# michelbarbeau/gr-uwspr

Hardware: NVIDIA B200
Metric: WSPR windows/sec (coarse+fine sync+demod) (higher is better)
Workload: dtype f32

## Files before the change

### gr-uwspr_b200/csrc/capi.cu

```cuda
#include <limits.h>
#include <math.h>
#include <stdio.h>
#include <stdlib.h>
#include <string.h>

#include <algorithm>
#include <chrono>
#include <future>
#include <string>
#include <thread>
#include <vector>

#include "common.cuh"
#include "../host/wspr_tables.h"

#ifndef M_PI
#define M_PI 3.14159265358979323846
#endif

namespace {

const int kMaxChunks = 1024;
const int kCounterSets = 15;
const int kCounterInts = 4 + 4 * kCounterSets;

struct UwChunk {
    int w0, nw, set, slot, cset, group, strm;
    size_t xoff;
};

struct Knobs {
    int host_chunk = 0;
    int tail_groups = 2;
    int tail_piece = 0;
    bool no_tail_split = false;
    bool no_early_d2h = false;
    bool trace = false;
    bool no_fine_reuse = false;
    int dev_chunks = 1;
    int fine_ctas_per_sm = 0;
    int fine_slice = 16384;
    int fine_slice_side = 16384;
};

Knobs read_knobs()
{
    Knobs k;
    auto geti = [](const char *name, int def) {
        const char *e = getenv(name);
        return e ? atoi(e) : def;
    };
    k.host_chunk = std::max(0, geti("UWSPR_B200_HOST_CHUNK", k.host_chunk));
    k.tail_groups = std::max(0, std::min(2, geti("UWSPR_B200_TAIL_GROUPS", k.tail_groups)));
    k.tail_piece = std::max(0, geti("UWSPR_B200_TAIL_PIECE", 0));
    k.no_tail_split = getenv("UWSPR_B200_NO_TAIL_SPLIT") != nullptr;
    k.no_early_d2h = getenv("UWSPR_B200_NO_EARLY_D2H") != nullptr;
    k.trace = getenv("UWSPR_B200_TRACE") != nullptr;
    k.no_fine_reuse = getenv("UWSPR_B200_NO_FINE_REUSE") != nullptr;
    k.dev_chunks = std::max(1, geti("UWSPR_B200_DEV_CHUNKS", 1));
    k.fine_ctas_per_sm = std::max(0, geti("UWSPR_B200_FINE_CTAS_PER_SM", 0));
    k.fine_slice = std::max(1, geti("UWSPR_B200_FINE_SLICE", k.fine_slice));
    k.fine_slice_side = std::max(1, geti("UWSPR_B200_FINE_SLICE_SIDE", k.fine_slice_side));
    return k;
}

struct Buffers {
    float2 *x_stage[3] = { nullptr, nullptr, nullptr };
    size_t x_stage_elems = 0;
    float *amp = nullptr;
    float *ps_dbg = nullptr;
    float *psavg = nullptr;
    UwPeak *peaks = nullptr;
    int *npk = nullptr;
    int *base = nullptr;
    size_t win_cap = 0;
    UwItem *items = nullptr;
    uwspr_b200_candidate_t *cands = nullptr;
    uwspr_b200_refined_t *refined = nullptr;
    uwspr_b200_jiggle_t *jig = nullptr;
    uint8_t *soft = nullptr;
    int *fine_tickets = nullptr;
    void *fine_state[3] = { nullptr, nullptr, nullptr };
    void *fine_pbuf[3] = { nullptr, nullptr, nullptr };
    void *fine_pe[3] = { nullptr, nullptr, nullptr };
    void *fine_pbest[3] = { nullptr, nullptr, nullptr };
    void *fine_tables[3] = { nullptr, nullptr, nullptr };
    int *counters = nullptr;
    float *window = nullptr;
    float2 *twiddle = nullptr;
    uint32_t *off4 = nullptr;
    short *hyp_unique = nullptr;
    int *dec_first_ok = nullptr;
    int *dec_tasks = nullptr;
    uint32_t *dec_task_cycles = nullptr;
    unsigned long long *dec_task_msg = nullptr;
    int *dec_counters = nullptr;
    uint8_t *dec_out = nullptr;
    short *mettab = nullptr;
    uint8_t *rows = nullptr;
    size_t rows_cap = 0;
};

}

struct uwspr_b200_ctx {
    uwspr_b200_params_t prm;
    UwDims d;
    Buffers b;
    int device = 0, sm_count = 0;
    int chunk_windows = 0, max_windows = 0, max_candidates = 0;
    int grid_coarse = 0, grid_points = 0, grid_lags = 0;
    int fine_slice[3] = { 0, 0, 0 };
    cudaStream_t compute = nullptr, compute2 = nullptr, compute3 = nullptr, copy = nullptr, d2h = nullptr;
    int *h_ends = nullptr;
    bool own_compute = true;
    cudaEvent_t ev_h2d[3] = { nullptr, nullptr, nullptr }, ev_free[3] = { nullptr, nullptr, nullptr }, ev_wl[3] = { nullptr, nullptr, nullptr };
    cudaEvent_t ev_fork = nullptr, ev_join = nullptr, ev_join3 = nullptr;
    int last_cw = 0;
    std::vector<UwChunk> last_chunks;
    Knobs knobs;
    int last_sets = 1;
    std::vector<cudaEvent_t> ev;
    cudaEvent_t ev_begin = nullptr, ev_end = nullptr;
    cudaEvent_t ev_cp0 = nullptr, ev_cp1 = nullptr, ev_kend = nullptr;
    float ms[4] = { 0, 0, 0, 0 };
    int64_t launches = 0;
    std::string err;
    bool debug_ps = false;
    bool have_coarse = false;
    bool have_fine = false;
    int last_jig_count = 0;
    int fano_grid = 0;
    int last_nwin = 0, last_total = 0;
    const float *last_samples = nullptr;
    int64_t last_stride = 0;
    std::future<int> pending;
};

namespace {

int fail(uwspr_b200_ctx *c, int status, const std::string &msg)
{
    if (c) c->err = msg;
    return status;
// ... 274 lines not shown
        const float2 *xfine = xdev + uw_window_offset(geom, 0);
        const size_t so = (size_t)s * cw + (size_t)ch.slot;
        float *amp = b.amp + so * d.n_rows * d.nbp;
        float *psd = (ctx->debug_ps && b.ps_dbg) ? b.ps_dbg + so * d.n_rows * d.nbp : nullptr;
        float *psavg = b.psavg + so * d.nbp;
        UwPeak *peaks = b.peaks + so * d.maxcand;
        int *set = b.counters + 4 + 4 * ch.cset;
        cudaEvent_t *e = &ctx->ev[4 * c];
        CU(cudaEventRecord(e[0], st));
        if (do_coarse) {
            uw_launch_spectrogram(d, xdev, geom, nw, b.window, b.twiddle, amp, psd, psavg, peaks,
                                  b.npk + w0, st);
            ctx->launches++;
        }
        CU(cudaEventRecord(e[1], st));
        if (c >= 1 && chunks[c - 1].strm != ch.strm) CU(cudaStreamWaitEvent(st, ctx->ev_wl[chunks[c - 1].strm], 0));
        uw_launch_worklist(b.npk + w0, nw, ctx->max_candidates, b.base + w0, b.items, b.counters, set, st);
        ctx->launches++;
        if (streams[1] != cs) CU(cudaEventRecord(ctx->ev_wl[ch.strm], st));
        if (early) CU(cudaMemcpyAsync(&ctx->h_ends[c], set + 2, sizeof(int), cudaMemcpyDeviceToHost, st));
        if (do_coarse) {
            uw_launch_coarse(d, amp, peaks, b.items, set + 2, ctx->max_candidates, b.off4, b.hyp_unique, b.cands, set,
                             ctx->grid_coarse, st);
            ctx->launches++;
        }
        CU(cudaEventRecord(e[2], st));
        if (do_fine) {
            const long long most = std::min<long long>(ctx->max_candidates, (long long)nw * d.maxcand);
            const int slice = ctx->fine_slice[ch.strm];
            for (long long s0 = 0; s0 < most; s0 += slice)
                ctx->launches += uw_launch_fine(d, xfine, geom, b.items, set + 1, set + 2, ctx->max_candidates, b.cands,
                                                jig_first, jig_count, b.refined, b.jig, b.soft, (int)s0, slice,
                                                b.fine_state[ch.strm], b.fine_pbuf[ch.strm], b.fine_pe[ch.strm], b.fine_pbest[ch.strm], b.fine_tables[ch.strm], b.fine_tickets + 16 * ch.strm, ctx->grid_points,
                                                ctx->grid_lags, kn.no_fine_reuse ? 0 : 1, st);
        }
        CU(cudaEventRecord(e[3], st));
        if (host) CU(cudaEventRecord(ctx->ev_free[s], st));
    }
    if (streams[1] != cs) {
        CU(cudaEventRecord(ctx->ev_join, streams[1]));
        CU(cudaStreamWaitEvent(cs, ctx->ev_join, 0));
        if (use3) {
            CU(cudaEventRecord(ctx->ev_join3, streams[2]));
            CU(cudaStreamWaitEvent(cs, ctx->ev_join3, 0));
        }
    }
    ctx->last_cw = cw;
    ctx->last_sets = nsets;
    if (ctx->knobs.trace) CU(cudaEventRecord(ctx->ev_kend, cs));
    int done = 0;
    auto fetch = [&](int lo, int hi, cudaStream_t q) -> cudaError_t {
        cudaError_t e = cudaSuccess;
        const size_t n = (size_t)(hi - lo);
        if (hi <= lo) return e;
        if (cands_out && do_coarse && e == cudaSuccess)
            e = cudaMemcpyAsync(cands_out + lo, b.cands + lo, sizeof(uwspr_b200_candidate_t) * n, cudaMemcpyDeviceToHost, q);
        if (do_fine && refined_out && e == cudaSuccess)
            e = cudaMemcpyAsync(refined_out + lo, b.refined + lo, sizeof(uwspr_b200_refined_t) * n, cudaMemcpyDeviceToHost, q);
        if (do_fine && jig_out && e == cudaSuccess)
            e = cudaMemcpyAsync(jig_out + (size_t)lo * jig_count, b.jig + (size_t)lo * jig_count,
                                sizeof(uwspr_b200_jiggle_t) * n * jig_count, cudaMemcpyDeviceToHost, q);
        if (do_fine && soft_out && e == cudaSuccess)
            e = cudaMemcpyAsync(soft_out + (size_t)lo * jig_count * UW_NSYM, b.soft + (size_t)lo * jig_count * UW_NSYM,
                                n * jig_count * UW_NSYM, cudaMemcpyDeviceToHost, q);
        return e;
    };
    if (early) {
// ... 182 lines not shown
    }
    CUC(cudaMalloc(&b.window, UW_FFT_N * sizeof(float)));
    CUC(cudaMalloc(&b.twiddle, UW_FFT_N * sizeof(float2)));
    CUC(cudaMalloc(&b.off4, off4.size() * sizeof(uint32_t)));
    CUC(cudaMalloc(&b.hyp_unique, hyp_unique.size() * sizeof(short)));
    CUC(cudaMemcpy(b.window, window.data(), UW_FFT_N * sizeof(float), cudaMemcpyHostToDevice));
    CUC(cudaMemcpy(b.twiddle, tw.data(), UW_FFT_N * sizeof(float2), cudaMemcpyHostToDevice));
    CUC(cudaMemcpy(b.off4, off4.data(), off4.size() * sizeof(uint32_t), cudaMemcpyHostToDevice));
    CUC(cudaMemcpy(b.hyp_unique, hyp_unique.data(), hyp_unique.size() * sizeof(short), cudaMemcpyHostToDevice));
    CUC(cudaStreamCreateWithFlags(&ctx->compute, cudaStreamNonBlocking));
    CUC(cudaStreamCreateWithFlags(&ctx->copy, cudaStreamNonBlocking));
    CUC(cudaStreamCreateWithFlags(&ctx->compute2, cudaStreamNonBlocking));
    CUC(cudaStreamCreateWithFlags(&ctx->d2h, cudaStreamNonBlocking));
    CUC(cudaStreamCreateWithFlags(&ctx->compute3, cudaStreamNonBlocking));
    CUC(cudaEventCreateWithFlags(&ctx->ev_join3, cudaEventDisableTiming));
    CUC(cudaHostAlloc(&ctx->h_ends, sizeof(int) * (kMaxChunks + 4), cudaHostAllocDefault));
    CUC(cudaEventCreateWithFlags(&ctx->ev_fork, cudaEventDisableTiming));
    CUC(cudaEventCreateWithFlags(&ctx->ev_join, cudaEventDisableTiming));
    for (int q = 0; q < 3; q++) {
        CUC(cudaEventCreateWithFlags(&ctx->ev_h2d[q], cudaEventDisableTiming));
        CUC(cudaEventCreateWithFlags(&ctx->ev_free[q], cudaEventDisableTiming));
        CUC(cudaEventCreateWithFlags(&ctx->ev_wl[q], cudaEventDisableTiming));
    }
    CUC(cudaEventCreate(&ctx->ev_begin));
    CUC(cudaEventCreate(&ctx->ev_cp0));
    CUC(cudaEventCreate(&ctx->ev_cp1));
    CUC(cudaEventCreate(&ctx->ev_kend));
    CUC(cudaEventCreate(&ctx->ev_end));
    if (uw_coarse_setup(d) || uw_fine_setup() || uw_fano_setup())
        return bail(fail(ctx, UWSPR_B200_E_CUDA, "cannot reserve shared memory for the kernels (not an sm_100a device?)"));
    ctx->grid_coarse = ctx->sm_count * uw_coarse_blocks_per_sm(d);
    ctx->fano_grid = ctx->sm_count * uw_fano_blocks_per_sm();
    {
        int bp = 1, bl = 1;
        uw_fine_blocks_per_sm(&bp, &bl);
        if (ctx->knobs.fine_ctas_per_sm > 0) {
            bp = std::min(bp, ctx->knobs.fine_ctas_per_sm);
            bl = std::min(bl, ctx->knobs.fine_ctas_per_sm);
        }
        ctx->grid_points = ctx->sm_count * bp;
        ctx->grid_lags = ctx->sm_count * bl;
        if (ctx->knobs.trace)
            fprintf(stderr, "uwspr_b200 trace: fine path: %d + %d resident CTAs per SM (points, lags), slices of %d candidates\n", bp, bl,
                    std::max(1, std::min(ctx->max_candidates, ctx->knobs.fine_slice)));
    }
    CUC(cudaDeviceSynchronize());
#undef CUC
    *ctx_out = ctx;
    return UWSPR_B200_OK;
}

void uwspr_b200_destroy(uwspr_b200_ctx *ctx)
{
    if (!ctx) return;
    if (ctx->pending.valid()) ctx->pending.wait();
    cudaSetDevice(ctx->device);
    Buffers &b = ctx->b;
    void *ptrs[] = { b.x_stage[0], b.x_stage[1], b.x_stage[2], b.amp, b.ps_dbg, b.psavg, b.peaks, b.npk, b.base, b.items,
                     b.cands, b.refined, b.jig, b.soft, b.counters, b.fine_tickets, b.fine_state[0], b.fine_state[1], b.fine_state[2], b.fine_pbuf[0], b.fine_pbuf[1],
                     b.fine_pbuf[2], b.fine_pe[0], b.fine_pe[1], b.fine_pe[2], b.fine_pbest[0], b.fine_pbest[1], b.fine_pbest[2], b.fine_tables[0], b.fine_tables[1], b.fine_tables[2], b.window, b.twiddle, b.off4, b.hyp_unique,
                     b.dec_first_ok, b.dec_tasks, b.dec_task_cycles, b.dec_task_msg, b.dec_counters, b.dec_out, b.mettab, b.rows };
    for (void *q : ptrs)
        if (q) cudaFree(q);
    for (cudaEvent_t e : ctx->ev) cudaEventDestroy(e);
    for (int q = 0; q < 3; q++) {
        if (ctx->ev_h2d[q]) cudaEventDestroy(ctx->ev_h2d[q]);
        if (ctx->ev_free[q]) cudaEventDestroy(ctx->ev_free[q]);
        if (ctx->ev_wl[q]) cudaEventDestroy(ctx->ev_wl[q]);
    }
    if (ctx->ev_begin) cudaEventDestroy(ctx->ev_begin);
    if (ctx->ev_cp0) cudaEventDestroy(ctx->ev_cp0);
    if (ctx->ev_cp1) cudaEventDestroy(ctx->ev_cp1);
    if (ctx->ev_kend) cudaEventDestroy(ctx->ev_kend);
    if (ctx->ev_end) cudaEventDestroy(ctx->ev_end);
    if (ctx->compute && ctx->own_compute) cudaStreamDestroy(ctx->compute);
    if (ctx->copy) cudaStreamDestroy(ctx->copy);
    if (ctx->compute2) cudaStreamDestroy(ctx->compute2);
// ... 347 lines not shown
```

### gr-uwspr_b200/csrc/common.cuh

```cuda
#pragma once

#include <cuda_runtime.h>
#include <stdint.h>

#include "uwspr_b200.h"

#define UW_NSYM 162
#define UW_FFT_N 512
#define UW_HOP 128
#define UW_NK0 26
#define UW_NIFR 5
#define UW_NTRAJ 125
#define UW_SPS 256
#define UW_NP 45000
#define UW_MAX_TILE_W 40
#define UW_MAX_UNIQUE 192
#define UW_NQUAD 41

struct UwDims {
    int fl, n_rows, size, m, hpbm, finpb, noiseidx, maxfreqs, maxcand, maxdrift, cf;
    float df, min_snr, floor_val, threshold;
    int bin_lo, n_bins, nbp;
    int n_lin, n_hyp, n_unique;
    int off_min, off_max, tile_w;
// ... 55 lines not shown
}
__device__ __forceinline__ uw_f2 uw_sub2(uw_f2 a, uw_f2 b)
{
    uw_f2 r;
    asm("sub.rn.f32x2 %0, %1, %2;" : "=l"(r) : "l"(a), "l"(b));
    return r;
}
__device__ __forceinline__ uw_f2 uw_mul2(uw_f2 a, uw_f2 b, uw_f2 nz)
{
    uw_f2 r;
    asm("fma.rn.f32x2 %0, %1, %2, %3;" : "=l"(r) : "l"(a), "l"(b), "l"(nz));
    return r;
}
__device__ __forceinline__ uw_f2 uw_fma2(uw_f2 a, uw_f2 b, uw_f2 c)
{
    uw_f2 r;
    asm("fma.rn.f32x2 %0, %1, %2, %3;" : "=l"(r) : "l"(a), "l"(b), "l"(c));
    return r;
}
__device__ __forceinline__ uw_f2 uw_mul2s(float a, uw_f2 b, uw_f2 nz) { return uw_mul2(uw_pk(a, a), b, nz); }

void uw_launch_spectrogram(const UwDims &d, const float2 *x, const UwGeom &geom, int nwin,
                           const float *window, const float2 *twiddle, float *amp, float *ps_dbg,
                           float *psavg, UwPeak *peaks, int *npk, cudaStream_t s);
void uw_launch_worklist(const int *npk, int nwin, int cap, int *base, UwItem *items, int *counters,
                        int *set, cudaStream_t s);
void uw_launch_coarse(const UwDims &d, const float *amp, const UwPeak *peaks, const UwItem *items,
                      const int *total, int cap, const uint32_t *off4, const short *hyp_unique,
                      uwspr_b200_candidate_t *cands, int *ticket, int grid, cudaStream_t s);
int uw_launch_fine(const UwDims &d, const float2 *x, const UwGeom &geom, const UwItem *items, const int *begin,
                   const int *end, int cap, const uwspr_b200_candidate_t *cands, int jig_first, int jig_count,
                   uwspr_b200_refined_t *refined, uwspr_b200_jiggle_t *jig, uint8_t *soft, int slice0, int slice_n,
                   void *state, void *pbuf, void *pE, void *pbest, void *tables, int *tickets, int grid_points, int grid_lags,
                   int reuse, cudaStream_t s);
int uw_coarse_fine_channels(uwspr_b200_ctx *ctx, const float *samples, int64_t win_stride, int wins_per_chan,
                            int64_t chan_stride, int nchan, int jig_first, int jig_count, int32_t *npk,
                            uwspr_b200_candidate_t *cands, int cap, int32_t *total);
int64_t uw_frontend_stream_launches(const uwspr_b200_frontend_stream *s);
size_t uw_fine_state_bytes();
size_t uw_fine_pbuf_bytes();
size_t uw_fine_pe_bytes();
size_t uw_fine_pbest_bytes();
size_t uw_fine_tables_bytes();
void uw_fine_blocks_per_sm(int *points, int *lags);
size_t uw_coarse_smem_bytes(const UwDims &d);
int uw_coarse_setup(const UwDims &d);
int uw_fine_setup();
int uw_coarse_blocks_per_sm(const UwDims &d);
void uw_launch_fano_candidates(const uwspr_b200_refined_t *refined, const uwspr_b200_jiggle_t *jig, const uint8_t *soft,
                               int ncand, int jig_count, const short *mettab, int *first_ok, int *tasks, int *counters,
                               uint32_t *task_cycles, unsigned long long *task_msg, int grid, uint8_t *decoded,
                               int8_t *msg7, int32_t *idt_used, uint32_t *fano_cycles, cudaStream_t s);
void uw_launch_fano_rows(const uint8_t *symbols, int n, int nbits, int delta, uint32_t maxcycles, const short *mettab,
                         int32_t *status, uint32_t *metric, uint32_t *cycles, uint32_t *maxnp, uint8_t *data11, cudaStream_t s);
int uw_fano_setup();
int uw_fano_blocks_per_sm();
```

### gr-uwspr_b200/csrc/fine.cu

```cuda
#include "common.cuh"

namespace {

constexpr int kThreads = 256;
constexpr int kWarps = kThreads / 32;
constexpr int kPB = 5;
constexpr int kKC1 = 8;
constexpr int kPitch1 = kKC1 + 2;
constexpr int kNChunk1 = UW_SPS / kKC1;
constexpr int kRows2 = 32;
constexpr int kPass2 = UW_NSYM / kRows2;
constexpr int kSpan2 = 128;
constexpr int kKCR = 32;
constexpr int kRing = kSpan2 + 2 * kKCR;
constexpr int kPitch2 = kRing + 1;
constexpr int kMaxJ = UWSPR_B200_NJIG;
constexpr int kLagPT = 5;
constexpr int kMemo = 24;
#ifndef LAGS_CTAS
#define LAGS_CTAS 3
#endif
#ifndef RING_UNROLL
#define RING_UNROLL 1
#endif
constexpr int kRingUnroll = RING_UNROLL;
constexpr size_t kWarpSmem = 2 * 32 * kPitch1 * sizeof(float2) + 2 * 2 * kKC1 * 2 * sizeof(float4);
constexpr int kSlots1 = (kPB * UW_NSYM + 31) / 32;
constexpr int kSlotsRest = (kMaxJ * (UW_NSYM - kPass2 * kRows2) + 31) / 32;
#ifndef UW_R1_FAST
#define UW_R1_FAST 1
#endif
#ifndef UW_R1_LDS128
#define UW_R1_LDS128 1
#endif

struct FineCand {
    float f1, drift1, sync1;
    int shift1;
    int worth;
    int npt, nev;
    float pt_f0[kPB];
    int pt_lag[kPB];
    float pt_drift[kPB];
    float pt_ss[kPB];
    int ev[kPB];
    int tab[kPB];
    int ntab;
    float tab_f0[kPB], tab_drift[kPB];
    int memo_n;
    float memo_f0[kMemo], memo_drift[kMemo], memo_ss[kMemo];
    int memo_lag[kMemo];
// ... 271 lines not shown
#undef UW_STAGEF_ALL
#undef UW_STAGE_TABLE
    if (live)
        *out = make_float4(tone_mag(uw_lo(inp[0]), uw_lo(quad[0])), tone_mag(uw_hi(inp[0]), uw_hi(quad[0])),
                           tone_mag(uw_lo(inp[1]), uw_lo(quad[1])), tone_mag(uw_hi(inp[1]), uw_hi(quad[1])));
}

__global__ void __launch_bounds__(128) k_fine_tables(FineArgs a)
{
    const int n = slice_count(a);
    const int begin = *a.begin_ptr + a.slice0;
    const int gt = blockIdx.x * blockDim.x + threadIdx.x;
    const int cidx = gt / 32, t = (gt % 32) >> 2, j = gt & 3;
    if (cidx >= n || t >= kPB) return;
    const FineCand &st = a.st[cidx];
    if (t >= st.ntab) return;
    const uwspr_b200_candidate_t cand = load_cand(a.cands, begin + cidx);
    const float fp = symbol_freq(a.d, cand, st.tab_f0[t], st.tab_drift[t], 0);
    float cd, sd;
    tone_seed(a.fc, fp, j, cd, sd);
    float c = 1.0f, s = 0.0f;
    float *out = reinterpret_cast<float *>(a.tables + ((size_t)cidx * kPB + t) * (UW_SPS * 2)) + 4 * (j >> 1) + (j & 1);
    for (int k = 0; k < UW_SPS; k++) {
        out[8 * k] = c;
        out[8 * k + 2] = s;
        const float cn = __fsub_rn(__fmul_rn(c, cd), __fmul_rn(s, sd));
        const float sn = __fadd_rn(__fmul_rn(c, sd), __fmul_rn(s, cd));
        c = cn;
        s = sn;
    }
}

template <bool REST>
__global__ void __launch_bounds__(kThreads, 4) k_fine_points(FineArgs a, int tk)
{
    extern __shared__ __align__(16) unsigned char smem_raw[];
    const int lane = threadIdx.x & 31, warp = threadIdx.x >> 5;
    WarpTile xt = reinterpret_cast<WarpTile>(smem_raw + (size_t)warp * kWarpSmem);
    TableTile tt = reinterpret_cast<TableTile>(smem_raw + (size_t)warp * kWarpSmem + 2 * 32 * kPitch1 * sizeof(float2));
    const int n = slice_count(a);
    const int begin = *a.begin_ptr + a.slice0;
    constexpr int kSlots = REST ? kSlotsRest : kSlots1;
    constexpr int s_lo = REST ? kPass2 * kRows2 : 0, s_cnt = REST ? UW_NSYM - kPass2 * kRows2 : UW_NSYM;
    for (;;) {
        int slot = 0;
        if (lane == 0) slot = atomicAdd(a.tickets + tk, 1);
        slot = __shfl_sync(0xffffffffu, slot, 0);
        if (slot >= n * kSlots) break;
        const int cidx = slot / kSlots, local = slot - cidx * kSlots;
        const FineCand &st = a.st[cidx];
        const int np = REST ? (st.worth == 1 ? st.nl : 0) : st.nev;
        const int ntask = np * s_cnt;
        if (local * 32 >= ntask) continue;
        const int g = begin + cidx;
        const uwspr_b200_candidate_t cand = load_cand(a.cands, g);
        const float2 *xw = a.x + st.xoff;
        const int task = local * 32 + lane;
        const bool live = task < ntask;
        const int tq = min(task, ntask - 1);
        const int q = tq / s_cnt;
        const int i = s_lo + (tq - q * s_cnt);
        float f0, drift;
        int lag, tab = -1;
        float4 *out;
        if (REST) {
            f0 = st.e_f0;
            drift = st.e_drift;
            lag = st.e_lag[q];
            out = a.pE + ((size_t)cidx * UW_NSYM + i) * kMaxJ + q;
        } else {
            const int pq = st.ev[q];
            f0 = st.pt_f0[pq];
            drift = st.pt_drift[pq];
            lag = st.pt_lag[pq];
            tab = st.tab[q];
            out = a.pbuf + ((size_t)cidx * UW_NSYM + i) * kPB + q;
        }
        if (!REST && __all_sync(0xffffffffu, tab >= 0)) {
            const int tab_a = __shfl_sync(0xffffffffu, tab, 0), tab_b = __shfl_sync(0xffffffffu, tab, 31);
            const float4 *tbase = a.tables + (size_t)cidx * kPB * (UW_SPS * 2);
            r1_task<true>(xt, tt, a.d, a.fc, xw, cand, live, f0, drift, lag, i, tbase + (size_t)tab_a * (UW_SPS * 2),
                          tbase + (size_t)tab_b * (UW_SPS * 2), tab == tab_a ? 0 : 1, out);
        } else {
            r1_task<false>(xt, tt, a.d, a.fc, xw, cand, live, f0, drift, lag, i, nullptr, nullptr, 0, out);
// ... 118 lines not shown
                for (int r = warp; r < kRows2; r += kWarps) {
                    const int nn = lag_min + (i0 + r) * UW_SPS + t0 + lane;
                    const bool ok = (unsigned)(nn - 1) < (unsigned)(UW_NP - 1);
                    const unsigned sdst = (unsigned)__cvta_generic_to_shared(&sm.tile[r][slot0 + lane]);
                    cp_async8_s<0>(sdst, ok ? xw + nn : xw, ok ? 8 : 0);
                }
            }
            cp_async_commit();
            if (live) {
                if (ln == 5)
                    lag_chunk_ring<5>(ad, row_end, c, s, cd, sd, inp, quad, nz);
                else if (ln == 4)
                    lag_chunk_ring<4>(ad, row_end, c, s, cd, sd, inp, quad, nz);
                else if (ln == 3)
                    lag_chunk_ring<3>(ad, row_end, c, s, cd, sd, inp, quad, nz);
                else if (ln == 2)
                    lag_chunk_ring<2>(ad, row_end, c, s, cd, sd, inp, quad, nz);
                else
                    lag_chunk_ring<1>(ad, row_end, c, s, cd, sd, inp, quad, nz);
            }
            cp_async_wait<0>();
            __syncthreads();
        }
        if (live) {
            float2 *out = reinterpret_cast<float2 *>(a.pE + ((size_t)cidx * UW_NSYM + i) * kMaxJ) + tp;
#pragma unroll
            for (int l = 0; l < kLagPT; l++)
                if (l < ln)
                    out[2 * (l0 + l)] = make_float2(tone_mag(uw_lo(inp[l]), uw_lo(quad[l])), tone_mag(uw_hi(inp[l]), uw_hi(quad[l])));
        }
    }
}

__device__ __forceinline__ bool const_freq(bool lin, bool intended_t, float drift)
{
    return lin ? (drift == 0.0f) : !intended_t;
}

__device__ __forceinline__ void stage_points(FineCand &st, int np, bool lin, bool intended_t)
{
    int nev = 0;
    for (int q = 0; q < np; q++) {
        int hit = -1;
        for (int m = 0; m < st.memo_n; m++)
            if (__float_as_uint(st.memo_f0[m]) == __float_as_uint(st.pt_f0[q]) && st.memo_lag[m] == st.pt_lag[q] &&
                __float_as_uint(st.memo_drift[m]) == __float_as_uint(st.pt_drift[q])) {
                hit = m;
                break;
            }
        if (hit >= 0)
            st.pt_ss[q] = st.memo_ss[hit];
        else
            st.ev[nev++] = q;
    }
    st.npt = np;
    st.nev = nev;
    int ntab = 0;
    for (int e = 0; e < nev; e++) {
        const int q = st.ev[e];
        int t = -1;
        if (const_freq(lin, intended_t, st.pt_drift[q])) {
            for (int u = 0; u < ntab && t < 0; u++)
                if (__float_as_uint(st.tab_f0[u]) == __float_as_uint(st.pt_f0[q]) &&
                    __float_as_uint(st.tab_drift[u]) == __float_as_uint(st.pt_drift[q]))
                    t = u;
            if (t < 0) {
// ... 65 lines not shown
        static_assert(UW_NSYM % kBatch == 0, "162 = 18 x 9");
        for (int i0 = 0; i0 < UW_NSYM; i0 += kBatch) {
            float4 vb[kBatch];
#pragma unroll
            for (int k = 0; k < kBatch; k++) vb[k] = p[(size_t)(i0 + k) * kPB];
#pragma unroll
            for (int k = 0; k < kBatch; k++) {
                const float4 v = vb[k];
                totp = __fadd_rn(__fadd_rn(__fadd_rn(__fadd_rn(totp, v.x), v.y), v.z), v.w);
                const float cmet = __fsub_rn(__fadd_rn(v.y, v.w), __fadd_rn(v.x, v.z));
                ss = uw_sync_bit(a.d.sync_words, i0 + k) ? __fadd_rn(ss, cmet) : __fsub_rn(ss, cmet);
            }
        }
        st.pt_ss[st.ev[sub]] = __fdiv_rn(ss, totp);
    }
    __syncwarp(gmask);
    if (!have || skip) return;
    if (sub == 0) {
        const uwspr_b200_candidate_t cand = a.cands[g];
        const bool lin = cand.m_type == 0;
        if (STAGE == 0) {
            st.f1 = cand.freq;
            st.drift1 = lin ? cand.m_linear.drift : 0.0f;
            st.shift1 = cand.shift;
            st.sync1 = cand.sync;
            st.memo_n = 0;
            st.worth = -1;
            st.nl = 0;
            st.best_have = 0;
            st.best_col = -1;
            st.e_reuse = -1;
            st.xoff = (int)(uw_window_offset(a.geom, a.items[g].win) - uw_window_offset(a.geom, 0));
            if (cidx == 0)
                for (int q = 0; q < 8; q++) a.tickets[q] = 0;
        } else {
            for (int e = 0; e < st.nev && st.memo_n < kMemo; e++) {
                const int q = st.ev[e], m = st.memo_n++;
                st.memo_f0[m] = st.pt_f0[q];
                st.memo_lag[m] = st.pt_lag[q];
                st.memo_drift[m] = st.pt_drift[q];
                st.memo_ss[m] = st.pt_ss[q];
            }
        }
        if (STAGE == 1 || STAGE == 2 || STAGE == 4 || STAGE == 5) select_best(st);
        if (STAGE == 3) st.best_col = -1;
        if (STAGE == 3 && lin) {
            const float syncp = (st.pt_ss[0] > -1e30f) ? st.pt_ss[0] : -1e30f;
            const float syncm = (st.pt_ss[1] > -1e30f) ? st.pt_ss[1] : -1e30f;
            if (!(st.pt_ss[1] > -1e30f)) {
                st.f1 = 0.0f;
                st.shift1 = 0;
            }
            if (syncp > st.sync1) {
                st.drift1 = st.pt_drift[0];
                st.sync1 = syncp;
                keep_point(st, 0);
            } else if (syncm > st.sync1) {
                st.drift1 = st.pt_drift[1];
                st.sync1 = syncm;
                keep_point(st, 1);
            }
        }
        if (STAGE == 3) st.worth = (st.sync1 > minsync1) ? 1 : 0;
        const float f1 = st.f1, drift1 = st.drift1;
        const int shift1 = st.shift1;
        int np = 0;
        if (STAGE == 0 || STAGE == 3) {
// ... 143 lines not shown
        if (q < -128.0f) q = -128.0f;
        const float w = __fadd_rn(q, 128.0f);
        const int sym = (w == w) ? (int)w : 0;
        if (soft_g) soft_g[i] = (uint8_t)sym;
        const int y = (sym & 0xff) - 128;
        sq += y * y;
    }
    if (a.jig) {
        uwspr_b200_jiggle_t r;
        const float sy = (sync > -1e30f) ? sync : -1e30f;
        r.sync = sy;
        r.rms = (float)__dsqrt_rn(__ddiv_rn((double)(float)sq, 162.0));
        r.shift = kept ? st.shift1 : st.e_lag[slot];
        r.gate = (sy > minsync2 && r.rms > minrms) ? 1 : 0;
        a.jig[(long long)g * a.jig_count + jidx] = r;
    }
}

constexpr size_t kPointsSmem = (size_t)kWarps * kWarpSmem;

}

size_t uw_fine_state_bytes() { return sizeof(FineCand); }
size_t uw_fine_pbuf_bytes() { return (size_t)UW_NSYM * kPB * sizeof(float4); }
size_t uw_fine_pe_bytes() { return (size_t)UW_NSYM * kMaxJ * sizeof(float4); }
size_t uw_fine_pbest_bytes() { return (size_t)UW_NSYM * sizeof(float4); }
size_t uw_fine_tables_bytes() { return (size_t)kPB * UW_SPS * 2 * sizeof(float4); }

int uw_fine_setup()
{
    if (cudaFuncSetAttribute(k_fine_lags, cudaFuncAttributeMaxDynamicSharedMemorySize, (int)sizeof(LagSmem)) != cudaSuccess) return 1;
    if (cudaFuncSetAttribute(k_fine_points<false>, cudaFuncAttributeMaxDynamicSharedMemorySize, (int)kPointsSmem) != cudaSuccess) return 1;
    if (cudaFuncSetAttribute(k_fine_points<true>, cudaFuncAttributeMaxDynamicSharedMemorySize, (int)kPointsSmem) != cudaSuccess) return 1;
    return 0;
}

void uw_fine_blocks_per_sm(int *points, int *lags)
{
    int n = 0;
    *points = (cudaOccupancyMaxActiveBlocksPerMultiprocessor(&n, k_fine_points<false>, kThreads, kPointsSmem) == cudaSuccess && n > 0) ? n : 1;
    *lags = (cudaOccupancyMaxActiveBlocksPerMultiprocessor(&n, k_fine_lags, kThreads, sizeof(LagSmem)) == cudaSuccess && n > 0) ? n : 1;
}

int uw_launch_fine(const UwDims &d, const float2 *x, const UwGeom &geom, const UwItem *items, const int *begin,
                   const int *end, int cap, const uwspr_b200_candidate_t *cands, int jig_first, int jig_count,
                   uwspr_b200_refined_t *refined, uwspr_b200_jiggle_t *jig, uint8_t *soft, int slice0, int slice_n,
                   void *state, void *pbuf, void *pE, void *pbest, void *tables, int *tickets, int grid_points, int grid_lags,
                   int reuse, cudaStream_t s)
{
    FineArgs a;
    a.reuse = reuse;
    a.pbest = static_cast<float4 *>(pbest);
    a.tables = static_cast<float4 *>(tables);
    a.tickets = tickets;
    a.d = d;
    const float dt = (float)(1.0 / 375.0), df = (float)(375.0 / 256.0);
    a.fc.delta[0] = (float)(-df * 1.5);
    a.fc.delta[1] = (float)(-df * 0.5);
    a.fc.delta[2] = (float)(df * 0.5);
    a.fc.delta[3] = (float)(df * 1.5);
    a.fc.twopidt = 2 * 3.14159265358979323846 * dt;
    a.fc.nz = UW_NEGZERO2;
    a.x = x;
    a.geom = geom;
    a.items = items;
    a.cands = cands;
    a.begin_ptr = begin;
    a.end_ptr = end;
    a.cap = cap;
    a.slice0 = slice0;
    a.slice_n = slice_n;
    a.st = static_cast<FineCand *>(state);
    a.pbuf = static_cast<float4 *>(pbuf);
    a.pE = static_cast<float4 *>(pE);
    a.jig_first = jig_first;
    a.jig_count = jig_count;
    a.refined = refined;
    a.jig = jig;
    a.soft = soft;
    const int step_grid = (slice_n * 8 + 255) / 256;
    int launches = 0;
#define UW_STEP(S)                                         \
    k_fine_step<S><<<step_grid, 256, 0, s>>>(a);          \
    launches++
    int tk = 0;
#define UW_POINTS()                                                            \
    k_fine_tables<<<(slice_n * 32 + 127) / 128, 128, 0, s>>>(a);              \
    k_fine_points<false><<<grid_points, kThreads, kPointsSmem, s>>>(a, tk++); \
    launches += 2
    UW_STEP(0);
    UW_POINTS();
    UW_STEP(1);
    UW_POINTS();
    UW_STEP(2);
    UW_POINTS();
    UW_STEP(3);
    UW_POINTS();
    UW_STEP(4);
    UW_POINTS();
    UW_STEP(5);
#undef UW_STEP
#undef UW_POINTS
    if (jig_count > 0) {
        k_fine_lags<<<grid_lags, kThreads, sizeof(LagSmem), s>>>(a, tk++);
        k_fine_points<true><<<grid_points, kThreads, kPointsSmem, s>>>(a, tk++);
        k_fine_finish<<<(slice_n * 32 + 127) / 128, 128, 0, s>>>(a);
        launches += 3;
    }
    return launches;
}
```

Baseline: 322,700.

## Add lag-sharing fine-sync kernel that reuses staged samples across lag points

Adds a k_fine_lagshare kernel that handles the fine-sync evaluation points of steps 0 and 3 whose candidates differ only in lag (tab[0] < 0). It stages each symbol's samples into shared memory once with cp.async, either as double-buffered segments or as a ring, and accumulates several lag points from the same staged data. k_fine_points skips those candidates in those steps. The aim is to cut redundant global loads and per-point work in the points kernel, at the cost of two extra launches per slice and more complex staging code. The UWSPR_B200_NO_LAG_SHARE variable disables it.

```diff
diff --git a/gr-uwspr_b200/csrc/capi.cu b/gr-uwspr_b200/csrc/capi.cu
--- a/gr-uwspr_b200/csrc/capi.cu
+++ b/gr-uwspr_b200/csrc/capi.cu
@@ -37,6 +37,7 @@
     bool no_early_d2h = false;
     bool trace = false;
     bool no_fine_reuse = false;
+    bool no_lag_share = false;
     int dev_chunks = 1;
     int fine_ctas_per_sm = 0;
     int fine_slice = 16384;
@@ -57,6 +58,7 @@
     k.no_early_d2h = getenv("UWSPR_B200_NO_EARLY_D2H") != nullptr;
     k.trace = getenv("UWSPR_B200_TRACE") != nullptr;
     k.no_fine_reuse = getenv("UWSPR_B200_NO_FINE_REUSE") != nullptr;
+    k.no_lag_share = getenv("UWSPR_B200_NO_LAG_SHARE") != nullptr;
     k.dev_chunks = std::max(1, geti("UWSPR_B200_DEV_CHUNKS", 1));
     k.fine_ctas_per_sm = std::max(0, geti("UWSPR_B200_FINE_CTAS_PER_SM", 0));
     k.fine_slice = std::max(1, geti("UWSPR_B200_FINE_SLICE", k.fine_slice));
@@ -109,7 +111,7 @@
     Buffers b;
     int device = 0, sm_count = 0;
     int chunk_windows = 0, max_windows = 0, max_candidates = 0;
-    int grid_coarse = 0, grid_points = 0, grid_lags = 0;
+    int grid_coarse = 0, grid_points = 0, grid_lags = 0, grid_share = 0;
     int fine_slice[3] = { 0, 0, 0 };
     cudaStream_t compute = nullptr, compute2 = nullptr, compute3 = nullptr, copy = nullptr, d2h = nullptr;
     int *h_ends = nullptr;
@@ -450,7 +452,7 @@
                 ctx->launches += uw_launch_fine(d, xfine, geom, b.items, set + 1, set + 2, ctx->max_candidates, b.cands,
                                                 jig_first, jig_count, b.refined, b.jig, b.soft, (int)s0, slice,
                                                 b.fine_state[ch.strm], b.fine_pbuf[ch.strm], b.fine_pe[ch.strm], b.fine_pbest[ch.strm], b.fine_tables[ch.strm], b.fine_tickets + 16 * ch.strm, ctx->grid_points,
-                                                ctx->grid_lags, kn.no_fine_reuse ? 0 : 1, st);
+                                                ctx->grid_lags, ctx->grid_share, kn.no_fine_reuse ? 0 : 1, st);
         }
         CU(cudaEventRecord(e[3], st));
         if (host) CU(cudaEventRecord(ctx->ev_free[s], st));
@@ -699,17 +701,19 @@
     ctx->grid_coarse = ctx->sm_count * uw_coarse_blocks_per_sm(d);
     ctx->fano_grid = ctx->sm_count * uw_fano_blocks_per_sm();
     {
-        int bp = 1, bl = 1;
-        uw_fine_blocks_per_sm(&bp, &bl);
+        int bp = 1, bl = 1, bs = 1;
+        uw_fine_blocks_per_sm(&bp, &bl, &bs);
         if (ctx->knobs.fine_ctas_per_sm > 0) {
             bp = std::min(bp, ctx->knobs.fine_ctas_per_sm);
             bl = std::min(bl, ctx->knobs.fine_ctas_per_sm);
+            bs = std::min(bs, ctx->knobs.fine_ctas_per_sm);
         }
         ctx->grid_points = ctx->sm_count * bp;
         ctx->grid_lags = ctx->sm_count * bl;
+        ctx->grid_share = ctx->knobs.no_lag_share ? 0 : ctx->sm_count * bs;
         if (ctx->knobs.trace)
-            fprintf(stderr, "uwspr_b200 trace: fine path: %d + %d resident CTAs per SM (points, lags), slices of %d candidates\n", bp, bl,
-                    std::max(1, std::min(ctx->max_candidates, ctx->knobs.fine_slice)));
+            fprintf(stderr, "uwspr_b200 trace: fine path: %d + %d + %d resident CTAs per SM (points, lags, lag share%s), slices of %d candidates\n",
+                    bp, bl, bs, ctx->knobs.no_lag_share ? " off" : "", std::max(1, std::min(ctx->max_candidates, ctx->knobs.fine_slice)));
     }
     CUC(cudaDeviceSynchronize());
 #undef CUC
diff --git a/gr-uwspr_b200/csrc/common.cuh b/gr-uwspr_b200/csrc/common.cuh
--- a/gr-uwspr_b200/csrc/common.cuh
+++ b/gr-uwspr_b200/csrc/common.cuh
@@ -111,7 +111,7 @@
                    const int *end, int cap, const uwspr_b200_candidate_t *cands, int jig_first, int jig_count,
                    uwspr_b200_refined_t *refined, uwspr_b200_jiggle_t *jig, uint8_t *soft, int slice0, int slice_n,
                    void *state, void *pbuf, void *pE, void *pbest, void *tables, int *tickets, int grid_points, int grid_lags,
-                   int reuse, cudaStream_t s);
+                   int grid_share, int reuse, cudaStream_t s);
 int uw_coarse_fine_channels(uwspr_b200_ctx *ctx, const float *samples, int64_t win_stride, int wins_per_chan,
                             int64_t chan_stride, int nchan, int jig_first, int jig_count, int32_t *npk,
                             uwspr_b200_candidate_t *cands, int cap, int32_t *total);
@@ -121,7 +121,7 @@
 size_t uw_fine_pe_bytes();
 size_t uw_fine_pbest_bytes();
 size_t uw_fine_tables_bytes();
-void uw_fine_blocks_per_sm(int *points, int *lags);
+void uw_fine_blocks_per_sm(int *points, int *lags, int *share);
 size_t uw_coarse_smem_bytes(const UwDims &d);
 int uw_coarse_setup(const UwDims &d);
 int uw_fine_setup();
diff --git a/gr-uwspr_b200/csrc/fine.cu b/gr-uwspr_b200/csrc/fine.cu
--- a/gr-uwspr_b200/csrc/fine.cu
+++ b/gr-uwspr_b200/csrc/fine.cu
@@ -1,4 +1,7 @@
 #include "common.cuh"
+
+#include <algorithm>
+#include <cassert>
 
 namespace {
 
@@ -17,6 +20,7 @@
 constexpr int kMaxJ = UWSPR_B200_NJIG;
 constexpr int kLagPT = 5;
 constexpr int kMemo = 24;
+constexpr int kTickets = 16;
 #ifndef LAGS_CTAS
 #define LAGS_CTAS 3
 #endif
@@ -354,7 +358,7 @@
 }
 
 template <bool REST>
-__global__ void __launch_bounds__(kThreads, 4) k_fine_points(FineArgs a, int tk)
+__global__ void __launch_bounds__(kThreads, 4) k_fine_points(FineArgs a, int tk, int lag_share)
 {
     extern __shared__ __align__(16) unsigned char smem_raw[];
     const int lane = threadIdx.x & 31, warp = threadIdx.x >> 5;
@@ -371,7 +375,7 @@
         if (slot >= n * kSlots) break;
         const int cidx = slot / kSlots, local = slot - cidx * kSlots;
         const FineCand &st = a.st[cidx];
-        const int np = REST ? (st.worth == 1 ? st.nl : 0) : st.nev;
+        const int np = REST ? (st.worth == 1 ? st.nl : 0) : (lag_share && st.nev > 0 && st.tab[0] < 0) ? 0 : st.nev;
         const int ntask = np * s_cnt;
         if (local * 32 >= ntask) continue;
         const int g = begin + cidx;
@@ -556,6 +560,206 @@
     }
 }
 
+constexpr int kKS = 8;
+constexpr int kShareFull = UW_NSYM / 32;
+constexpr int kShareRestC = 16;
+constexpr int kStepA = 64, kStepD = 16;
+constexpr int kSegPitch = kKS + 1;
+constexpr int kSegB = 32 * kSegPitch * 8;
+constexpr int kShareBufB = kPB * kSegB;
+constexpr int kRingS = 4 * kStepD + 2 * kKS;
+constexpr int kRingPitch = kRingS + 1;
+constexpr int kShareWarpSmem = 2 * kShareBufB > 32 * kRingPitch * 8 ? 2 * kShareBufB : 32 * kRingPitch * 8;
+constexpr int kShareWarps = 2;
+constexpr int kShareThreads = 32 * kShareWarps;
+constexpr size_t kShareSmem = (size_t)kShareWarps * kShareWarpSmem;
+static_assert(kRingS % kKS == 0 && kStepD % kKS == 0 && UW_SPS % kKS == 0 && kKS == 8,
+              "a chunk of a lag never straddles the ring's wrap; eight lanes stage one row's chunk");
+
+template <bool RING, int NL>
+__device__ __forceinline__ void lagshare_run(unsigned wsm, const float2 *x, const float2 *const (&rp)[8], const int (&rb)[8],
+                                             const int (&pe)[kPB], uw_f2 (&cd)[2], uw_f2 (&sd)[2],
+                                             uw_f2 (&inp)[kPB][2], uw_f2 (&quad)[kPB][2], const uw_f2 nz)
+{
+    const int lane = threadIdx.x & 31, j = lane % kKS;
+    uw_f2 c[2], s[2], c2[2], s2[2];
+#pragma unroll
+    for (int t = 0; t < 2; t++) {
+        c[t] = uw_pk(1.0f, 1.0f);
+        s[t] = uw_pk(0.0f, 0.0f);
+    }
+    constexpr int kNChunk = UW_SPS / kKS;
+    int rsl[NL];
+    unsigned dst0;
+    if (RING) {
+        dst0 = wsm + (unsigned)((lane / kKS) * kRingPitch * 8 + j * 8);
+#pragma unroll
+        for (int e = 0; e < 8; e++)
+#pragma unroll
+            for (int q = 0; q < kRingS / kKS; q++) {
+                const int n_ = rb[e] + q * kKS;
+                const bool ok_ = (unsigned)(n_ - 1) < (unsigned)(UW_NP - 1);
+                asm volatile("cp.async.ca.shared.global [%0], [%1], 8, %2;\n" ::"r"(dst0 + (unsigned)(4 * e * kRingPitch * 8 + q * kKS * 8)),
+                             "l"(ok_ ? rp[e] + q * kKS : x), "r"(ok_ ? 8 : 0) : "memory");
+            }
+#pragma unroll
+        for (int l = 0; l < NL; l++) rsl[l] = kStepD * pe[l];
+    } else {
+        dst0 = wsm + (unsigned)((lane / kKS) * kSegPitch * 8 + j * 8);
+    }
+#define UW_SEG_STAGE(BUFOFF, CHUNK)                                                                              \
+    do {                                                                                                         \
+        _Pragma("unroll") for (int p = 0; p < kPB; p++)                                                          \
+        _Pragma("unroll") for (int e = 0; e < 8; e++) {                                                          \
+            const int o_ = kStepA * p + (CHUNK) * kKS;                                                           \
+            const int n_ = rb[e] + o_;                                                                           \
+            const bool ok_ = (unsigned)(n_ - 1) < (unsigned)(UW_NP - 1);                                         \
+            asm volatile("cp.async.ca.shared.global [%0], [%1], 8, %2;\n" ::"r"(dst0 + (BUFOFF) + (unsigned)(p * kSegB + 4 * e * kSegPitch * 8)), \
+                         "l"(ok_ ? rp[e] + o_ : x), "r"(ok_ ? 8 : 0) : "memory");                                \
+        }                                                                                                        \
+    } while (0)
+    if (!RING) UW_SEG_STAGE(0u, 0);
+    cp_async_commit();
+#pragma unroll 1
+    for (int k = 0; k < kNChunk; k++) {
+        if (RING) {
+            if (k >= 1 && k + 1 < kNChunk) {
+                const int t0 = k * kKS + kRingS - kKS;
+                const unsigned so = (unsigned)((t0 % kRingS) * 8);
+#pragma unroll
+                for (int e = 0; e < 8; e++) {
+                    const int n_ = rb[e] + t0;
+                    const bool ok_ = (unsigned)(n_ - 1) < (unsigned)(UW_NP - 1);
+                    asm volatile("cp.async.ca.shared.global [%0], [%1], 8, %2;\n" ::"r"(dst0 + so + (unsigned)(4 * e * kRingPitch * 8)),
+                                 "l"(ok_ ? rp[e] + t0 : x), "r"(ok_ ? 8 : 0) : "memory");
+                }
+            }
+        } else if (k + 1 < kNChunk) {
+            UW_SEG_STAGE((unsigned)(((k + 1) & 1) * kShareBufB), k + 1);
+        }
+        cp_async_commit();
+        cp_async_wait<1>();
+        __syncwarp();
+        unsigned ad[NL];
+#pragma unroll
+        for (int l = 0; l < NL; l++) {
+            if (RING) {
+                ad[l] = wsm + (unsigned)(lane * kRingPitch * 8 + rsl[l] * 8);
+                rsl[l] = rsl[l] + kKS == kRingS ? 0 : rsl[l] + kKS;
+            } else {
+                ad[l] = wsm + (unsigned)((k & 1) * kShareBufB + pe[l] * kSegB + lane * kSegPitch * 8);
+            }
+        }
+#pragma unroll 1
+        for (int h = 0; h < kKS / 4; h++) {
+#define UW_SHARE_STEP(Q, CN, SN, C, S)                                                   \
+    do {                                                                                 \
+        _Pragma("unroll") for (int l = 0; l < NL; l++) {                                 \
+            const float2 xv = lds_f2<8 * (Q)>(ad[l]);                                    \
+            UW_MAC2(inp[l][0], quad[l][0], xv, C[0], S[0]);                              \
+            UW_MAC2(inp[l][1], quad[l][1], xv, C[1], S[1]);                              \
+        }                                                                                \
+        UW_ROT2_TO(CN[0], SN[0], C[0], S[0], cd[0], sd[0]);                              \
+        UW_ROT2_TO(CN[1], SN[1], C[1], S[1], cd[1], sd[1]);                              \
+    } while (0)
+            UW_SHARE_STEP(0, c2, s2, c, s);
+            UW_SHARE_STEP(1, c, s, c2, s2);
+            UW_SHARE_STEP(2, c2, s2, c, s);
+            UW_SHARE_STEP(3, c, s, c2, s2);
+#undef UW_SHARE_STEP
+#pragma unroll
+            for (int l = 0; l < NL; l++) ad[l] += 4 * 8;
+        }
+        __syncwarp();
+    }
+    cp_async_wait<0>();
+#undef UW_SEG_STAGE
+}
+
+template <bool RING>
+__global__ void __launch_bounds__(kShareThreads, 4) k_fine_lagshare(FineArgs a, int tk)
+{
+    extern __shared__ __align__(16) unsigned char smem_raw[];
+    const int lane = threadIdx.x & 31, warp = threadIdx.x >> 5;
+    const unsigned wsm = (unsigned)__cvta_generic_to_shared(smem_raw) + (unsigned)(warp * kShareWarpSmem);
+    const int n = slice_count(a);
+    const int begin = *a.begin_ptr + a.slice0;
+    const int nfull = n * kShareFull;
+    const int nslots = nfull + (n + kShareRestC - 1) / kShareRestC;
+    const uw_f2 nz = a.fc.nz;
+    for (;;) {
+        int slot = 0;
+        if (lane == 0) slot = atomicAdd(a.tickets + tk, 1);
+        slot = __shfl_sync(0xffffffffu, slot, 0);
+        if (slot >= nslots) break;
+        int cidx, i;
+        if (slot < nfull) {
+            cidx = slot / kShareFull;
+            i = (slot - cidx * kShareFull) * 32 + lane;
+        } else {
+            cidx = (slot - nfull) * kShareRestC + lane / 2;
+            i = kShareFull * 32 + (lane & 1);
+        }
+        const FineCand &st = a.st[cidx < n ? cidx : 0];
+        const int nev = cidx < n ? st.nev : 0;
+        const bool live = nev > 0 && st.tab[0] < 0;
+        if (!__any_sync(0xffffffffu, live)) continue;
+        int nrow = -(1 << 28);
+        const float2 *xrow = a.x;
+        int pe[kPB];
+        uw_f2 cd[2] = { 0ull, 0ull }, sd[2] = { 0ull, 0ull };
+#pragma unroll
+        for (int e = 0; e < kPB; e++) pe[e] = 0;
+        if (live) {
+            const uwspr_b200_candidate_t cand = load_cand(a.cands, begin + cidx);
+#pragma unroll
+            for (int e = 0; e < kPB; e++) pe[e] = st.ev[e < nev ? e : 0];
+            const float fp = symbol_freq(a.d, cand, st.pt_f0[pe[0]], st.pt_drift[pe[0]], i);
+#pragma unroll
+            for (int t = 0; t < 2; t++) {
+                float cd0, sd0, cd1, sd1;
+                tone_seed(a.fc, fp, 2 * t, cd0, sd0);
+                tone_seed(a.fc, fp, 2 * t + 1, cd1, sd1);
+                cd[t] = uw_pk(cd0, cd1);
+                sd[t] = uw_pk(sd0, sd1);
+            }
+            nrow = st.pt_lag[0] + i * UW_SPS;
+            xrow = a.x + st.xoff;
+        }
+        int rb[8];
+        const float2 *rp[8];
+#pragma unroll
+        for (int e = 0; e < 8; e++) {
+            const int row = 4 * e + lane / kKS;
+            const int nr = __shfl_sync(0xffffffffu, nrow, row);
+            const unsigned long long pr = __shfl_sync(0xffffffffu, reinterpret_cast<unsigned long long>(xrow), row);
+            rb[e] = nr + lane % kKS;
+            rp[e] = reinterpret_cast<const float2 *>(pr) + (nr + lane % kKS);
+        }
+        uw_f2 inp[kPB][2], quad[kPB][2];
+#pragma unroll
+        for (int e = 0; e < kPB; e++)
+#pragma unroll
+            for (int t = 0; t < 2; t++) {
+                inp[e][t] = uw_pk(0.0f, 0.0f);
+                quad[e][t] = uw_pk(0.0f, 0.0f);
+            }
+        const int nl = __reduce_max_sync(0xffffffffu, live ? nev : 0);
+        if (!RING || nl == kPB)
+            lagshare_run<RING, kPB>(wsm, a.x, rp, rb, pe, cd, sd, inp, quad, nz);
+        else
+            lagshare_run<RING, kPB - 1>(wsm, a.x, rp, rb, pe, cd, sd, inp, quad, nz);
+        if (live) {
+            float4 *out = a.pbuf + ((size_t)cidx * UW_NSYM + i) * kPB;
+#pragma unroll
+            for (int e = 0; e < kPB; e++)
+                if (e < nev)
+                    out[e] = make_float4(tone_mag(uw_lo(inp[e][0]), uw_lo(quad[e][0])), tone_mag(uw_hi(inp[e][0]), uw_hi(quad[e][0])),
+                                         tone_mag(uw_lo(inp[e][1]), uw_lo(quad[e][1])), tone_mag(uw_hi(inp[e][1]), uw_hi(quad[e][1])));
+        }
+    }
+}
+
 __device__ __forceinline__ bool const_freq(bool lin, bool intended_t, float drift)
 {
     return lin ? (drift == 0.0f) : !intended_t;
@@ -687,7 +891,7 @@
             st.e_reuse = -1;
             st.xoff = (int)(uw_window_offset(a.geom, a.items[g].win) - uw_window_offset(a.geom, 0));
             if (cidx == 0)
-                for (int q = 0; q < 8; q++) a.tickets[q] = 0;
+                for (int q = 0; q < kTickets; q++) a.tickets[q] = 0;
         } else {
             for (int e = 0; e < st.nev && st.memo_n < kMemo; e++) {
                 const int q = st.ev[e], m = st.memo_n++;
@@ -897,21 +1101,26 @@
     if (cudaFuncSetAttribute(k_fine_lags, cudaFuncAttributeMaxDynamicSharedMemorySize, (int)sizeof(LagSmem)) != cudaSuccess) return 1;
     if (cudaFuncSetAttribute(k_fine_points<false>, cudaFuncAttributeMaxDynamicSharedMemorySize, (int)kPointsSmem) != cudaSuccess) return 1;
     if (cudaFuncSetAttribute(k_fine_points<true>, cudaFuncAttributeMaxDynamicSharedMemorySize, (int)kPointsSmem) != cudaSuccess) return 1;
+    if (cudaFuncSetAttribute(k_fine_lagshare<false>, cudaFuncAttributeMaxDynamicSharedMemorySize, (int)kShareSmem) != cudaSuccess) return 1;
+    if (cudaFuncSetAttribute(k_fine_lagshare<true>, cudaFuncAttributeMaxDynamicSharedMemorySize, (int)kShareSmem) != cudaSuccess) return 1;
     return 0;
 }
 
-void uw_fine_blocks_per_sm(int *points, int *lags)
-{
-    int n = 0;
+void uw_fine_blocks_per_sm(int *points, int *lags, int *share)
+{
+    int n = 0, m = 0;
     *points = (cudaOccupancyMaxActiveBlocksPerMultiprocessor(&n, k_fine_points<false>, kThreads, kPointsSmem) == cudaSuccess && n > 0) ? n : 1;
     *lags = (cudaOccupancyMaxActiveBlocksPerMultiprocessor(&n, k_fine_lags, kThreads, sizeof(LagSmem)) == cudaSuccess && n > 0) ? n : 1;
+    const bool ok = cudaOccupancyMaxActiveBlocksPerMultiprocessor(&n, k_fine_lagshare<false>, kShareThreads, kShareSmem) == cudaSuccess &&
+                    cudaOccupancyMaxActiveBlocksPerMultiprocessor(&m, k_fine_lagshare<true>, kShareThreads, kShareSmem) == cudaSuccess;
+    *share = (ok && std::min(n, m) > 0) ? std::min(n, m) : 1;
 }
 
 int uw_launch_fine(const UwDims &d, const float2 *x, const UwGeom &geom, const UwItem *items, const int *begin,
                    const int *end, int cap, const uwspr_b200_candidate_t *cands, int jig_first, int jig_count,
                    uwspr_b200_refined_t *refined, uwspr_b200_jiggle_t *jig, uint8_t *soft, int slice0, int slice_n,
                    void *state, void *pbuf, void *pE, void *pbest, void *tables, int *tickets, int grid_points, int grid_lags,
-                   int reuse, cudaStream_t s)
+                   int grid_share, int reuse, cudaStream_t s)
 {
     FineArgs a;
     a.reuse = reuse;
@@ -949,28 +1158,38 @@
     k_fine_step<S><<<step_grid, 256, 0, s>>>(a);          \
     launches++
     int tk = 0;
-#define UW_POINTS()                                                            \
-    k_fine_tables<<<(slice_n * 32 + 127) / 128, 128, 0, s>>>(a);              \
-    k_fine_points<false><<<grid_points, kThreads, kPointsSmem, s>>>(a, tk++); \
+    const int share = grid_share > 0 ? 1 : 0;
+#define UW_POINTS(LAGS)                                                                     \
+    k_fine_tables<<<(slice_n * 32 + 127) / 128, 128, 0, s>>>(a);                           \
+    k_fine_points<false><<<grid_points, kThreads, kPointsSmem, s>>>(a, tk++, LAGS && share); \
     launches += 2
     UW_STEP(0);
-    UW_POINTS();
+    UW_POINTS(1);
+    if (share) {
+        k_fine_lagshare<false><<<grid_share, kShareThreads, kShareSmem, s>>>(a, tk++);
+        launches++;
+    }
     UW_STEP(1);
-    UW_POINTS();
+    UW_POINTS(0);
     UW_STEP(2);
-    UW_POINTS();
+    UW_POINTS(0);
     UW_STEP(3);
-    UW_POINTS();
+    UW_POINTS(1);
+    if (share) {
+        k_fine_lagshare<true><<<grid_share, kShareThreads, kShareSmem, s>>>(a, tk++);
+        launches++;
+    }
     UW_STEP(4);
-    UW_POINTS();
+    UW_POINTS(0);
     UW_STEP(5);
 #undef UW_STEP
 #undef UW_POINTS
     if (jig_count > 0) {
         k_fine_lags<<<grid_lags, kThreads, sizeof(LagSmem), s>>>(a, tk++);
-        k_fine_points<true><<<grid_points, kThreads, kPointsSmem, s>>>(a, tk++);
+        k_fine_points<true><<<grid_points, kThreads, kPointsSmem, s>>>(a, tk++, 0);
         k_fine_finish<<<(slice_n * 32 + 127) / 128, 128, 0, s>>>(a);
         launches += 3;
     }
+    assert(tk <= kTickets);
     return launches;
 }
```

After: 338,900, median of 6. 1.05x the previous value.
